# zc402/video-classification

Measured on AMD Instinct MI355X. Metric: clips/sec SlowFast-R50 8x8, 32x224^2 bf16 training step, higher is better.
Workload: dtype bf16

## Files before the change

### video-classification_amd/csrc/bn_tail.hip

```cpp
#include "sfk_common.h"

namespace {

template <typename D> __device__ __forceinline__ float wload(const void* w, int64_t i) {
  return (float)static_cast<const D*>(w)[i];
}

constexpr int TF_CO = 8;
constexpr int TF_MAXC = 512;

__global__ __launch_bounds__(256) void bn_tail_fold_g_kernel(const float* __restrict__ parts, int nparts, int c, float* __restrict__ g) {
  const int ci = blockIdx.x * 4 + (threadIdx.x >> 6), lane = threadIdx.x & 63;
  if (ci >= c) return;
  double s = 0.0;
  for (int p = lane; p < nparts; p += 64) s += (double)parts[((int64_t)p * c + ci) * 2];
#pragma unroll
  for (int sft = 1; sft < 64; sft <<= 1) s += __shfl_xor(s, sft);
  if (lane == 0) g[ci] = (float)s;
}

template <typename D>
__global__ __launch_bounds__(256) void bn_tail_fwd_kernel(const float* __restrict__ gram, const float* __restrict__ gvec,
                                                          double n, int c, const void* w,
                                                          int cout, const float* gamma, const float* beta, float eps,
                                                          float momentum, float* running_mean, float* running_var,
                                                          int64_t* nbt, float* mean, float* invstd, float* scale,
                                                          float* shift, float* __restrict__ t, D* __restrict__ wd) {
  __shared__ float wl[TF_CO][TF_MAXC];
  __shared__ float gl[TF_MAXC];
  __shared__ double red[4 * TF_CO][2];
  __shared__ float acoef[TF_CO];
  const int co0 = blockIdx.x * TF_CO, tid = threadIdx.x;
  if (blockIdx.x == 0 && tid == 0 && nbt) nbt[0] += 1;
  const double inv_n = 1.0 / n;
  for (int i = tid; i < TF_CO * c; i += 256) {
    const int o = i / c, j = i % c;
    wl[o][j] = co0 + o < cout ? wload<D>(w, (int64_t)(co0 + o) * c + j) : 0.f;
  }
  for (int j = tid; j < c; j += 256) gl[j] = (float)((double)gvec[j] * inv_n);
  __syncthreads();
  constexpr int NR = TF_MAXC / 256;
  float acc[TF_CO][NR], accc[TF_CO][NR];
  double gbar[NR];
#pragma unroll
  for (int r = 0; r < NR; ++r) {
    const int ci = tid + 256 * r;
    gbar[r] = ci < c ? (double)gvec[ci] * inv_n : 0.0;
  }
#pragma unroll
  for (int o = 0; o < TF_CO; ++o)
#pragma unroll
    for (int r = 0; r < NR; ++r) { acc[o][r] = 0.f; accc[o][r] = 0.f; }
#pragma unroll 8
  for (int j = 0; j < c; ++j) {
    float gj[NR], gc[NR];
    const double mj = (double)gl[j];
#pragma unroll
    for (int r = 0; r < NR; ++r) {
      const int ci = tid + 256 * r;
      gj[r] = ci < c ? gram[(int64_t)j * c + ci] : 0.f;
      gc[r] = (float)((double)gj[r] * inv_n - mj * gbar[r]);
    }
#pragma unroll
    for (int o = 0; o < TF_CO; ++o) {
      const float wv = wl[o][j];
#pragma unroll
      for (int r = 0; r < NR; ++r) {
        acc[o][r] += wv * gj[r];
        accc[o][r] += wv * gc[r];
      }
    }
  }
  double p1[TF_CO], p2[TF_CO];
#pragma unroll
  for (int o = 0; o < TF_CO; ++o) {
    p1[o] = 0.0;
    p2[o] = 0.0;
#pragma unroll
    for (int r = 0; r < NR; ++r) {
      const int ci = tid + 256 * r;
      if (ci < c) {
        if (co0 + o < cout) t[(int64_t)(co0 + o) * c + ci] = acc[o][r];
        p1[o] += (double)wl[o][ci] * (double)gvec[ci];
        p2[o] += (double)accc[o][r] * (double)wl[o][ci];
      }
    }
#pragma unroll
    for (int sft = 1; sft < 64; sft <<= 1) {
      p1[o] += __shfl_xor(p1[o], sft);
      p2[o] += __shfl_xor(p2[o], sft);
    }
  }
  if ((tid & 63) == 0) {
#pragma unroll
    for (int o = 0; o < TF_CO; ++o) {
      red[(tid >> 6) * TF_CO + o][0] = p1[o];
      red[(tid >> 6) * TF_CO + o][1] = p2[o];
    }
  }
  __syncthreads();
  if (tid < TF_CO && co0 + tid < cout) {
    const int ch = co0 + tid;
    const double s1 = red[tid][0] + red[TF_CO + tid][0] + red[2 * TF_CO + tid][0] + red[3 * TF_CO + tid][0];
    const double s2 = red[tid][1] + red[TF_CO + tid][1] + red[2 * TF_CO + tid][1] + red[3 * TF_CO + tid][1];
    const double mu = s1 / n;
    double var = s2;
    if (var < 0.0) var = 0.0;
    const float is = (float)(1.0 / sqrt(var + (double)eps));
    const float sc = gamma[ch] * is;
    mean[ch] = (float)mu;
    invstd[ch] = is;
    scale[ch] = sc;
    shift[ch] = beta[ch] - (float)mu * sc;
    acoef[tid] = sc;
    if (running_mean) {
      const double unb = n > 1.0 ? var * n / (n - 1.0) : var;
      running_mean[ch] = (1.f - momentum) * running_mean[ch] + momentum * (float)mu;
      running_var[ch] = (1.f - momentum) * running_var[ch] + momentum * (float)unb;
    }
  }
  if (!wd) return;
  __syncthreads();
  for (int ci = tid; ci < c; ci += 256)
#pragma unroll
    for (int o = 0; o < TF_CO; ++o)
      if (co0 + o < cout) wd[(int64_t)ci * cout + co0 + o] = (D)(acoef[o] * wl[o][ci]);
}

template <typename D>
__global__ __launch_bounds__(256) void bn_tail_coef_kernel(const float* __restrict__ rx, const float* __restrict__ parts,
                                                           int nparts, double n, int c,
                                                           const void* w, int cout, const float* gamma,
                                                           const float* mean, const float* invstd, float* dgamma,
                                                           float* dbeta, float* coef) {
  const int co = blockIdx.x * 4 + (threadIdx.x >> 6), lane = threadIdx.x & 63;
  if (co >= cout) return;
  double sdy = 0.0;
#pragma unroll 4
  for (int ci = lane; ci < c; ci += 64) sdy += (double)wload<D>(w, (int64_t)co * c + ci) * (double)rx[(int64_t)co * c + ci];
  double s = 0.0;
#pragma unroll 8
  for (int p = lane; p < nparts; p += 64) s += (double)parts[((int64_t)p * cout + co) * 2];
#pragma unroll
  for (int sft = 1; sft < 64; sft <<= 1) {
    sdy += __shfl_xor(sdy, sft);
    s += __shfl_xor(s, sft);
  }
  if (lane != 0) return;
  const double is = (double)invstd[co], mu = (double)mean[co];
  const double sxh = is * (sdy - mu * s);
  dgamma[co] += (float)sxh;
  dbeta[co] += (float)s;
  const double A = (double)gamma[co] * is, c1 = s / n, c2 = sxh / n;
  coef[co * 4 + 0] = (float)A;
  coef[co * 4 + 1] = (float)(-A * c2 * is);
  coef[co * 4 + 2] = (float)(A * (c2 * is * mu - c1));
  coef[co * 4 + 3] = 0.f;
}

template <typename D>
__device__ __forceinline__ void bn_tail_apply_part(int bx, int by, const float* __restrict__ rx, const float* __restrict__ gvec,
                                                   const float* __restrict__ t, int c, int cout,
                                                   const float* __restrict__ coef, float* dw) {
  const int co0 = by * 32, ci0 = bx * 32;
  const int tx = threadIdx.x & 31, ty = threadIdx.x >> 5;
#pragma unroll
  for (int i = 0; i < 4; ++i) {
    const int co = co0 + ty + 8 * i, ci = ci0 + tx;
    if (co < cout && ci < c) {
      const float A = coef[co * 4], B = coef[co * 4 + 1], Cc = coef[co * 4 + 2];
      const int64_t idx = (int64_t)co * c + ci;
      dw[idx] += A * rx[idx] + B * t[idx] + Cc * gvec[ci];
    }
  }
}

template <typename D>
__device__ __forceinline__ void bn_tail_m_part(int bx, int by, const void* w, int c, int cout, const float* __restrict__ coef, D* m) {
  __shared__ float wi[16][17], wj[16][17], bco[16];
  const int tx = threadIdx.x & 15, ty = threadIdx.x >> 4;
  const int i = by * 16 + ty, j = bx * 16 + tx;
  float acc = 0.f;
  for (int co0 = 0; co0 < cout; co0 += 16) {
    const int co = co0 + ty;
    const int ci = by * 16 + tx, cj = bx * 16 + tx;
    wi[ty][tx] = (co < cout && ci < c) ? wload<D>(w, (int64_t)co * c + ci) : 0.f;
    wj[ty][tx] = (co < cout && cj < c) ? wload<D>(w, (int64_t)co * c + cj) : 0.f;
    if (threadIdx.x < 16) bco[threadIdx.x] = co0 + threadIdx.x < cout ? coef[(co0 + threadIdx.x) * 4 + 1] : 0.f;
    __syncthreads();
#pragma unroll
    for (int q = 0; q < 16; ++q) acc += bco[q] * wi[q][ty] * wj[q][tx];
    __syncthreads();
  }
  if (i < c && j < c) m[(int64_t)i * c + j] = (D)acc;
}

template <typename D>
__device__ __forceinline__ void bn_tail_bias_part(int bx, const void* w, int c, int cout, const float* __restrict__ coef,
                                                  float* bias) {
  __shared__ double red[16][17];
  const int col = threadIdx.x & 15, part = threadIdx.x >> 4;
  const int ci = bx * 16 + col;
  double s = 0.0;
  if (ci < c) {
#pragma unroll 4
    for (int co = part; co < cout; co += 16) s += (double)coef[co * 4 + 2] * (double)wload<D>(w, (int64_t)co * c + ci);
  }
  red[part][col] = s;
  __syncthreads();
  if (part == 0 && ci < c) {
    double a = 0.0;
#pragma unroll
    for (int p = 0; p < 16; ++p) a += red[p][col];
    bias[ci] = (float)a;
  }
}

template <typename D>
__global__ __launch_bounds__(256) void bn_tail_post_kernel(const float* rx, const float* gvec, const float* t, int c,
                                                           const void* w, int cout, const float* coef, float* dw, D* m,
                                                           float* bias, int ax, int nap, int mx, int nm) {
  int b = blockIdx.x;
  if (b < nap) { bn_tail_apply_part<D>(b % ax, b / ax, rx, gvec, t, c, cout, coef, dw); return; }
  b -= nap;
  if (b < nm) { bn_tail_m_part<D>(b % mx, b / mx, w, c, cout, coef, m); return; }
  bn_tail_bias_part<D>(b - nm, w, c, cout, coef, bias);
}

inline bool tail_args_ok(int c, int cout, int dtype) {
  return c > 0 && cout > 0 && (dtype == SFK_F32 || dtype == SFK_BF16);
}

}

extern "C" int sfk_bn_tail_fwd(const float* gram, const float* a_sums, int32_t a_nparts, int64_t count, float* g, int32_t c,
                               const void* w, int32_t w_dtype, int32_t cout,
                               const float* gamma, const float* beta, float eps, float momentum, float* running_mean,
                               float* running_var, int64_t* nbt, float* mean, float* invstd, float* scale, float* shift,
                               float* t, void* wd, sfk_stream_t stream) {
  if (!gram || !a_sums || a_nparts <= 0 || count <= 0 || !g || !w || !gamma || !beta || !mean || !invstd || !scale || !shift || !t)
    return SFK_ERR_INVALID;
  if (!tail_args_ok(c, cout, w_dtype) || (!running_mean) != (!running_var)) return SFK_ERR_INVALID;
  if (c > TF_MAXC) return SFK_ERR_UNSUPPORTED;
  hipStream_t s = static_cast<hipStream_t>(stream);
  hipLaunchKernelGGL(bn_tail_fold_g_kernel, dim3((c + 3) / 4), dim3(256), 0, s, a_sums, a_nparts, c, g);
  const dim3 grid((cout + TF_CO - 1) / TF_CO), blk(256);
  if (w_dtype == SFK_BF16)
    hipLaunchKernelGGL(bn_tail_fwd_kernel<bf16_t>, grid, blk, 0, s, gram, g, (double)count, c, w, cout, gamma, beta, eps, momentum,
                       running_mean, running_var, nbt, mean, invstd, scale, shift, t, static_cast<bf16_t*>(wd));
  else
    hipLaunchKernelGGL(bn_tail_fwd_kernel<float>, grid, blk, 0, s, gram, g, (double)count, c, w, cout, gamma, beta, eps, momentum,
                       running_mean, running_var, nbt, mean, invstd, scale, shift, t, static_cast<float*>(wd));
  SFK_CHECK_LAUNCH();
  return SFK_OK;
}

template <typename D>
static int tail_bwd_launch(const float* rx, const float* parts, int nparts, const float* g, int64_t count, const float* t, int c, const void* w, int cout,
                           const float* gamma, const float* mean, const float* invstd, float* dgamma, float* dbeta,
                           float* dw, void* m, float* bias, float* coef, hipStream_t s) {
  hipLaunchKernelGGL(bn_tail_coef_kernel<D>, dim3((cout + 3) / 4), dim3(256), 0, s, rx, parts, nparts, (double)count, c, w, cout, gamma, mean,
                     invstd, dgamma, dbeta, coef);
  const int ax = (c + 31) / 32, ay = (cout + 31) / 32, mx = (c + 15) / 16, nb = (c + 15) / 16;
  hipLaunchKernelGGL(bn_tail_post_kernel<D>, dim3(ax * ay + mx * mx + nb), dim3(256), 0, s, rx, g, t, c, w, cout, coef, dw,
                     static_cast<D*>(m), bias, ax, ax * ay, mx, mx * mx);
  SFK_CHECK_LAUNCH();
  return SFK_OK;
}

extern "C" int sfk_bn_tail_bwd(const float* rx, const float* parts, int32_t nparts, const float* g, int64_t count, const float* t,
                               int32_t c, const void* w, int32_t w_dtype, int32_t cout, const float* gamma, const float* mean, const float* invstd,
                               float* dgamma, float* dbeta, float* dw, void* m, float* bias, float* coef,
                               sfk_stream_t stream) {
  if (!rx || !parts || nparts <= 0 || !g || count <= 0 || !t || !w || !gamma || !mean || !invstd || !dgamma || !dbeta || !dw || !m || !bias || !coef)
    return SFK_ERR_INVALID;
  if (!tail_args_ok(c, cout, w_dtype)) return SFK_ERR_INVALID;
  hipStream_t s = static_cast<hipStream_t>(stream);
  return w_dtype == SFK_BF16
             ? tail_bwd_launch<bf16_t>(rx, parts, nparts, g, count, t, c, w, cout, gamma, mean, invstd, dgamma, dbeta, dw, m, bias, coef, s)
             : tail_bwd_launch<float>(rx, parts, nparts, g, count, t, c, w, cout, gamma, mean, invstd, dgamma, dbeta, dw, m, bias, coef, s);
}
```

Before: 1167.

## Use fp32 MFMA for BN-tail gram products and coalesce partial-sum folds

Rewrites the BN-tail forward W·Gram product and the backward W^T·diag(B)·W product to use 16x16x4 fp32 MFMA instructions, with register double-buffered gram loads and templated column tiling chosen by channel count. The partial-sum fold kernels now reduce 8 channels per block with 32 loads in flight per thread, replacing one-wave-per-channel strided reads. The post-kernel block order is also changed so the heavier M blocks are scheduled first. The cost targeted is scalar FMA throughput and poorly coalesced reads in these small BN-tail kernels. In exchange the code is more complex, and accumulating in fp32 MFMA may change rounding order.

```diff
diff --git a/video-classification_amd/csrc/bn_tail.hip b/video-classification_amd/csrc/bn_tail.hip
--- a/video-classification_amd/csrc/bn_tail.hip
+++ b/video-classification_amd/csrc/bn_tail.hip
@@ -6,125 +6,181 @@
   return (float)static_cast<const D*>(w)[i];
 }
 
-constexpr int TF_CO = 8;
+constexpr int TF_CO = 16;
 constexpr int TF_MAXC = 512;
+constexpr int FOLD_CH = 8;
+constexpr int FOLD_RG = 32;
+
+__device__ __forceinline__ f32x4 mma4(float a, float b, const f32x4& acc) {
+  return __builtin_amdgcn_mfma_f32_16x16x4f32(a, b, acc, 0, 0, 0);
+}
+
+constexpr int FOLD_U = 32;
+struct FoldRegs { float v[FOLD_U]; };
+__device__ __forceinline__ void fold_issue(const float* __restrict__ parts, int nparts, int nch, int ch, int p0, FoldRegs& f) {
+#pragma unroll
+  for (int u = 0; u < FOLD_U; ++u) {
+    const int p = p0 + u * FOLD_RG;
+    f.v[u] = (ch < nch && p < nparts) ? parts[((int64_t)p * nch + ch) * 2] : 0.f;
+  }
+}
+__device__ __forceinline__ double fold_sum(const FoldRegs& f) {
+  double s = 0.0;
+#pragma unroll
+  for (int u = 0; u < FOLD_U; ++u) s += (double)f.v[u];
+  return s;
+}
+__device__ __forceinline__ double fold_rows(const float* __restrict__ parts, int nparts, int nch, int ch0, const FoldRegs& first) {
+  __shared__ double fred[4][FOLD_CH];
+  const int tid = threadIdx.x, chl = tid & (FOLD_CH - 1), rg = tid / FOLD_CH, ch = ch0 + chl;
+  double s = fold_sum(first);
+  for (int p0 = rg + FOLD_U * FOLD_RG; p0 < nparts; p0 += FOLD_U * FOLD_RG) {
+    FoldRegs f;
+    fold_issue(parts, nparts, nch, ch, p0, f);
+    s += fold_sum(f);
+  }
+#pragma unroll
+  for (int sft = FOLD_CH; sft < 64; sft <<= 1) s += __shfl_xor(s, sft);
+  if ((tid & 63) < FOLD_CH) fred[tid >> 6][chl] = s;
+  __syncthreads();
+  return tid < FOLD_CH ? (fred[0][tid] + fred[1][tid]) + (fred[2][tid] + fred[3][tid]) : 0.0;
+}
 
 __global__ __launch_bounds__(256) void bn_tail_fold_g_kernel(const float* __restrict__ parts, int nparts, int c, float* __restrict__ g) {
-  const int ci = blockIdx.x * 4 + (threadIdx.x >> 6), lane = threadIdx.x & 63;
-  if (ci >= c) return;
-  double s = 0.0;
-  for (int p = lane; p < nparts; p += 64) s += (double)parts[((int64_t)p * c + ci) * 2];
-#pragma unroll
-  for (int sft = 1; sft < 64; sft <<= 1) s += __shfl_xor(s, sft);
-  if (lane == 0) g[ci] = (float)s;
-}
-
-template <typename D>
+  const int ch0 = blockIdx.x * FOLD_CH;
+  FoldRegs f;
+  fold_issue(parts, nparts, c, ch0 + (threadIdx.x & (FOLD_CH - 1)), threadIdx.x / FOLD_CH, f);
+  const double s = fold_rows(parts, nparts, c, ch0, f);
+  const int ci = ch0 + threadIdx.x;
+  if (threadIdx.x < FOLD_CH && ci < c) g[ci] = (float)s;
+}
+
+template <typename D, int NT>
 __global__ __launch_bounds__(256) void bn_tail_fwd_kernel(const float* __restrict__ gram, const float* __restrict__ gvec,
                                                           double n, int c, const void* w,
                                                           int cout, const float* gamma, const float* beta, float eps,
                                                           float momentum, float* running_mean, float* running_var,
                                                           int64_t* nbt, float* mean, float* invstd, float* scale,
                                                           float* shift, float* __restrict__ t, D* __restrict__ wd) {
-  __shared__ float wl[TF_CO][TF_MAXC];
-  __shared__ float gl[TF_MAXC];
-  __shared__ double red[4 * TF_CO][2];
+  constexpr int CP = 64 * NT, LD = CP + 4;
+  constexpr int KU = NT <= 2 ? 16 : 32 / NT;
+  constexpr int KP = NT == 1 ? 2 : 1;
+  __shared__ float wl[TF_CO][LD];
+  __shared__ double gd[CP];
+  __shared__ double red[4][TF_CO];
+  __shared__ double mus[TF_CO];
   __shared__ float acoef[TF_CO];
-  const int co0 = blockIdx.x * TF_CO, tid = threadIdx.x;
+  const int tid = threadIdx.x, wave = tid >> 6, l = tid & 63, lr = l & 15, lq = l >> 4;
+  const int co0 = blockIdx.x * TF_CO;
   if (blockIdx.x == 0 && tid == 0 && nbt) nbt[0] += 1;
   const double inv_n = 1.0 / n;
-  for (int i = tid; i < TF_CO * c; i += 256) {
-    const int o = i / c, j = i % c;
-    wl[o][j] = co0 + o < cout ? wload<D>(w, (int64_t)(co0 + o) * c + j) : 0.f;
-  }
-  for (int j = tid; j < c; j += 256) gl[j] = (float)((double)gvec[j] * inv_n);
-  __syncthreads();
-  constexpr int NR = TF_MAXC / 256;
-  float acc[TF_CO][NR], accc[TF_CO][NR];
-  double gbar[NR];
-#pragma unroll
-  for (int r = 0; r < NR; ++r) {
-    const int ci = tid + 256 * r;
-    gbar[r] = ci < c ? (double)gvec[ci] * inv_n : 0.0;
-  }
-#pragma unroll
-  for (int o = 0; o < TF_CO; ++o)
-#pragma unroll
-    for (int r = 0; r < NR; ++r) { acc[o][r] = 0.f; accc[o][r] = 0.f; }
-#pragma unroll 8
-  for (int j = 0; j < c; ++j) {
-    float gj[NR], gc[NR];
-    const double mj = (double)gl[j];
-#pragma unroll
-    for (int r = 0; r < NR; ++r) {
-      const int ci = tid + 256 * r;
-      gj[r] = ci < c ? gram[(int64_t)j * c + ci] : 0.f;
-      gc[r] = (float)((double)gj[r] * inv_n - mj * gbar[r]);
-    }
-#pragma unroll
-    for (int o = 0; o < TF_CO; ++o) {
-      const float wv = wl[o][j];
-#pragma unroll
-      for (int r = 0; r < NR; ++r) {
-        acc[o][r] += wv * gj[r];
-        accc[o][r] += wv * gc[r];
+  const int ksteps = (c + 3) >> 2;
+  int col[NT];
+  double gbc[NT];
+#pragma unroll
+  for (int q = 0; q < NT; ++q) {
+    col[q] = 16 * (wave + 4 * q) + lr;
+    gbc[q] = col[q] < c ? (double)gvec[col[q]] * inv_n : 0.0;
+  }
+  const bool fin = tid < TF_CO && co0 + tid < cout;
+  const float gam = fin ? gamma[co0 + tid] : 0.f, bet = fin ? beta[co0 + tid] : 0.f;
+  const float rm0 = (fin && running_mean) ? running_mean[co0 + tid] : 0.f, rv0 = (fin && running_mean) ? running_var[co0 + tid] : 0.f;
+  float gcur[KU][NT], gnxt[KU][NT];
+  auto load_g = [&](const int s0, float (&gr)[KU][NT]) __attribute__((always_inline)) {
+#pragma unroll
+    for (int u = 0; u < KU; ++u) {
+      const int k = 4 * (s0 + u) + lq;
+#pragma unroll
+      for (int q = 0; q < NT; ++q) gr[u][q] = (k < c && col[q] < c) ? gram[(int64_t)k * c + col[q]] : 0.f;
+    }
+  };
+  load_g(0, gcur);
+  for (int i = tid; i < TF_CO * CP; i += 256) {
+    const int o = i / CP, j = i % CP;
+    wl[o][j] = (co0 + o < cout && j < c) ? wload<D>(w, (int64_t)(co0 + o) * c + j) : 0.f;
+  }
+  for (int j = tid; j < CP; j += 256) gd[j] = j < c ? (double)gvec[j] * inv_n : 0.0;
+  __syncthreads();
+  f32x4 acc[KP][NT], accc[KP][NT];
+#pragma unroll
+  for (int p = 0; p < KP; ++p)
+#pragma unroll
+    for (int q = 0; q < NT; ++q)
+#pragma unroll
+      for (int i = 0; i < 4; ++i) { acc[p][q][i] = 0.f; accc[p][q][i] = 0.f; }
+  for (int s0 = 0; s0 < ksteps; s0 += KU) {
+    const bool more = s0 + KU < ksteps;
+    if (more) load_g(s0 + KU, gnxt);
+#pragma unroll
+    for (int u = 0; u < KU; ++u) {
+      const int k = 4 * (s0 + u) + lq;
+      const float a = wl[lr][k];
+      const double mk = gd[k];
+#pragma unroll
+      for (int q = 0; q < NT; ++q) {
+        const float gj = gcur[u][q];
+        const float gc = (float)((double)gj * inv_n - mk * gbc[q]);
+        acc[u % KP][q] = mma4(a, gj, acc[u % KP][q]);
+        accc[u % KP][q] = mma4(a, gc, accc[u % KP][q]);
       }
     }
-  }
-  double p1[TF_CO], p2[TF_CO];
-#pragma unroll
-  for (int o = 0; o < TF_CO; ++o) {
-    p1[o] = 0.0;
-    p2[o] = 0.0;
-#pragma unroll
-    for (int r = 0; r < NR; ++r) {
-      const int ci = tid + 256 * r;
-      if (ci < c) {
-        if (co0 + o < cout) t[(int64_t)(co0 + o) * c + ci] = acc[o][r];
-        p1[o] += (double)wl[o][ci] * (double)gvec[ci];
-        p2[o] += (double)accc[o][r] * (double)wl[o][ci];
-      }
-    }
-#pragma unroll
-    for (int sft = 1; sft < 64; sft <<= 1) {
-      p1[o] += __shfl_xor(p1[o], sft);
-      p2[o] += __shfl_xor(p2[o], sft);
-    }
-  }
-  if ((tid & 63) == 0) {
-#pragma unroll
-    for (int o = 0; o < TF_CO; ++o) {
-      red[(tid >> 6) * TF_CO + o][0] = p1[o];
-      red[(tid >> 6) * TF_CO + o][1] = p2[o];
-    }
-  }
-  __syncthreads();
-  if (tid < TF_CO && co0 + tid < cout) {
+    if (more) {
+#pragma unroll
+      for (int u = 0; u < KU; ++u)
+#pragma unroll
+        for (int q = 0; q < NT; ++q) gcur[u][q] = gnxt[u][q];
+    }
+  }
+  double p2[4] = {0.0, 0.0, 0.0, 0.0};
+#pragma unroll
+  for (int q = 0; q < NT; ++q)
+#pragma unroll
+    for (int i = 0; i < 4; ++i) {
+      const int row = 4 * lq + i;
+      float tv = acc[0][q][i], tc = accc[0][q][i];
+      if constexpr (KP == 2) { tv += acc[1][q][i]; tc += accc[1][q][i]; }
+      if (co0 + row < cout && col[q] < c) t[(int64_t)(co0 + row) * c + col[q]] = tv;
+      p2[i] += (double)tc * (double)wl[row][col[q]];
+    }
+#pragma unroll
+  for (int i = 0; i < 4; ++i) {
+#pragma unroll
+    for (int sft = 1; sft < 16; sft <<= 1) p2[i] += __shfl_xor(p2[i], sft);
+    if (lr == 0) red[wave][4 * lq + i] = p2[i];
+  }
+  {
+    const int row = tid >> 4;
+    double s = 0.0;
+    for (int ci = lr; ci < c; ci += 16) s += (double)wl[row][ci] * gd[ci];
+#pragma unroll
+    for (int sft = 1; sft < 16; sft <<= 1) s += __shfl_xor(s, sft);
+    if (lr == 0) mus[row] = s;
+  }
+  __syncthreads();
+  if (fin) {
     const int ch = co0 + tid;
-    const double s1 = red[tid][0] + red[TF_CO + tid][0] + red[2 * TF_CO + tid][0] + red[3 * TF_CO + tid][0];
-    const double s2 = red[tid][1] + red[TF_CO + tid][1] + red[2 * TF_CO + tid][1] + red[3 * TF_CO + tid][1];
-    const double mu = s1 / n;
-    double var = s2;
+    const double mu = mus[tid];
+    double var = red[0][tid] + red[1][tid] + red[2][tid] + red[3][tid];
     if (var < 0.0) var = 0.0;
     const float is = (float)(1.0 / sqrt(var + (double)eps));
-    const float sc = gamma[ch] * is;
+    const float sc = gam * is;
     mean[ch] = (float)mu;
     invstd[ch] = is;
     scale[ch] = sc;
-    shift[ch] = beta[ch] - (float)mu * sc;
+    shift[ch] = bet - (float)mu * sc;
     acoef[tid] = sc;
     if (running_mean) {
       const double unb = n > 1.0 ? var * n / (n - 1.0) : var;
-      running_mean[ch] = (1.f - momentum) * running_mean[ch] + momentum * (float)mu;
-      running_var[ch] = (1.f - momentum) * running_var[ch] + momentum * (float)unb;
+      running_mean[ch] = (1.f - momentum) * rm0 + momentum * (float)mu;
+      running_var[ch] = (1.f - momentum) * rv0 + momentum * (float)unb;
     }
   }
   if (!wd) return;
   __syncthreads();
-  for (int ci = tid; ci < c; ci += 256)
-#pragma unroll
-    for (int o = 0; o < TF_CO; ++o)
-      if (co0 + o < cout) wd[(int64_t)ci * cout + co0 + o] = (D)(acoef[o] * wl[o][ci]);
+  for (int i = tid; i < c * TF_CO; i += 256) {
+    const int ci = i / TF_CO, o = i % TF_CO;
+    if (co0 + o < cout) wd[(int64_t)ci * cout + co0 + o] = (D)(acoef[o] * wl[o][ci]);
+  }
 }
 
 template <typename D>
@@ -133,25 +189,33 @@
                                                            const void* w, int cout, const float* gamma,
                                                            const float* mean, const float* invstd, float* dgamma,
                                                            float* dbeta, float* coef) {
-  const int co = blockIdx.x * 4 + (threadIdx.x >> 6), lane = threadIdx.x & 63;
-  if (co >= cout) return;
-  double sdy = 0.0;
+  __shared__ double sd[FOLD_CH];
+  const int co0 = blockIdx.x * FOLD_CH, tid = threadIdx.x;
+  FoldRegs f;
+  fold_issue(parts, nparts, cout, co0 + (tid & (FOLD_CH - 1)), tid / FOLD_CH, f);
+  const bool fin = tid < FOLD_CH && co0 + tid < cout;
+  const float isf = fin ? invstd[co0 + tid] : 0.f, muf = fin ? mean[co0 + tid] : 0.f, gam = fin ? gamma[co0 + tid] : 0.f;
+  const float dg0 = fin ? dgamma[co0 + tid] : 0.f, db0 = fin ? dbeta[co0 + tid] : 0.f;
+  {
+    const int co = co0 + (tid >> 5), j = tid & 31;
+    double a = 0.0;
+    if (co < cout) {
 #pragma unroll 4
-  for (int ci = lane; ci < c; ci += 64) sdy += (double)wload<D>(w, (int64_t)co * c + ci) * (double)rx[(int64_t)co * c + ci];
-  double s = 0.0;
-#pragma unroll 8
-  for (int p = lane; p < nparts; p += 64) s += (double)parts[((int64_t)p * cout + co) * 2];
-#pragma unroll
-  for (int sft = 1; sft < 64; sft <<= 1) {
-    sdy += __shfl_xor(sdy, sft);
-    s += __shfl_xor(s, sft);
-  }
-  if (lane != 0) return;
-  const double is = (double)invstd[co], mu = (double)mean[co];
+      for (int ci = j; ci < c; ci += 32) a += (double)wload<D>(w, (int64_t)co * c + ci) * (double)rx[(int64_t)co * c + ci];
+    }
+#pragma unroll
+    for (int sft = 1; sft < 32; sft <<= 1) a += __shfl_xor(a, sft);
+    if (j == 0) sd[tid >> 5] = a;
+  }
+  const double s = fold_rows(parts, nparts, cout, co0, f);
+  if (!fin) return;
+  const int co = co0 + tid;
+  const double sdy = sd[tid];
+  const double is = (double)isf, mu = (double)muf;
   const double sxh = is * (sdy - mu * s);
-  dgamma[co] += (float)sxh;
-  dbeta[co] += (float)s;
-  const double A = (double)gamma[co] * is, c1 = s / n, c2 = sxh / n;
+  dgamma[co] = dg0 + (float)sxh;
+  dbeta[co] = db0 + (float)s;
+  const double A = (double)gam * is, c1 = s / n, c2 = sxh / n;
   coef[co * 4 + 0] = (float)A;
   coef[co * 4 + 1] = (float)(-A * c2 * is);
   coef[co * 4 + 2] = (float)(A * (c2 * is * mu - c1));
@@ -177,22 +241,46 @@
 
 template <typename D>
 __device__ __forceinline__ void bn_tail_m_part(int bx, int by, const void* w, int c, int cout, const float* __restrict__ coef, D* m) {
-  __shared__ float wi[16][17], wj[16][17], bco[16];
-  const int tx = threadIdx.x & 15, ty = threadIdx.x >> 4;
-  const int i = by * 16 + ty, j = bx * 16 + tx;
-  float acc = 0.f;
-  for (int co0 = 0; co0 < cout; co0 += 16) {
-    const int co = co0 + ty;
-    const int ci = by * 16 + tx, cj = bx * 16 + tx;
-    wi[ty][tx] = (co < cout && ci < c) ? wload<D>(w, (int64_t)co * c + ci) : 0.f;
-    wj[ty][tx] = (co < cout && cj < c) ? wload<D>(w, (int64_t)co * c + cj) : 0.f;
-    if (threadIdx.x < 16) bco[threadIdx.x] = co0 + threadIdx.x < cout ? coef[(co0 + threadIdx.x) * 4 + 1] : 0.f;
-    __syncthreads();
-#pragma unroll
-    for (int q = 0; q < 16; ++q) acc += bco[q] * wi[q][ty] * wj[q][tx];
-    __syncthreads();
-  }
-  if (i < c && j < c) m[(int64_t)i * c + j] = (D)acc;
+  constexpr int KU = 16;
+  __shared__ float part[3][64][4];
+  const int tid = threadIdx.x, wave = tid >> 6, l = tid & 63, lr = l & 15, lq = l >> 4;
+  const int i = by * 16 + lr, j = bx * 16 + lr;
+  const int ksteps = (cout + 3) >> 2, per = (ksteps + 3) >> 2;
+  const int s_end = min(ksteps, (wave + 1) * per);
+  f32x4 acc[4];
+#pragma unroll
+  for (int p = 0; p < 4; ++p)
+#pragma unroll
+    for (int e = 0; e < 4; ++e) acc[p][e] = 0.f;
+  for (int s0 = wave * per; s0 < s_end; s0 += KU) {
+    float av[KU], bv[KU];
+#pragma unroll
+    for (int u = 0; u < KU; ++u) {
+      const int co = 4 * (s0 + u) + lq;
+      const bool ok = s0 + u < s_end && co < cout;
+      const float b = ok ? coef[co * 4 + 1] : 0.f;
+      const float wi = (ok && i < c) ? wload<D>(w, (int64_t)co * c + i) : 0.f;
+      av[u] = b * wi;
+      bv[u] = (ok && j < c) ? wload<D>(w, (int64_t)co * c + j) : 0.f;
+    }
+#pragma unroll
+    for (int u = 0; u < KU; ++u) acc[u & 3] = mma4(av[u], bv[u], acc[u & 3]);
+  }
+  f32x4 sum;
+#pragma unroll
+  for (int e = 0; e < 4; ++e) sum[e] = (acc[0][e] + acc[1][e]) + (acc[2][e] + acc[3][e]);
+  if (wave > 0) {
+#pragma unroll
+    for (int e = 0; e < 4; ++e) part[wave - 1][l][e] = sum[e];
+  }
+  __syncthreads();
+  if (wave > 0) return;
+#pragma unroll
+  for (int e = 0; e < 4; ++e) {
+    const float v = ((sum[e] + part[0][l][e]) + part[1][l][e]) + part[2][l][e];
+    const int row = by * 16 + 4 * lq + e;
+    if (row < c && j < c) m[(int64_t)row * c + j] = (D)v;
+  }
 }
 
 template <typename D>
@@ -203,7 +291,7 @@
   const int ci = bx * 16 + col;
   double s = 0.0;
   if (ci < c) {
-#pragma unroll 4
+#pragma unroll 8
     for (int co = part; co < cout; co += 16) s += (double)coef[co * 4 + 2] * (double)wload<D>(w, (int64_t)co * c + ci);
   }
   red[part][col] = s;
@@ -221,10 +309,10 @@
                                                            const void* w, int cout, const float* coef, float* dw, D* m,
                                                            float* bias, int ax, int nap, int mx, int nm) {
   int b = blockIdx.x;
+  if (b < nm) { bn_tail_m_part<D>(b % mx, b / mx, w, c, cout, coef, m); return; }
+  b -= nm;
   if (b < nap) { bn_tail_apply_part<D>(b % ax, b / ax, rx, gvec, t, c, cout, coef, dw); return; }
-  b -= nap;
-  if (b < nm) { bn_tail_m_part<D>(b % mx, b / mx, w, c, cout, coef, m); return; }
-  bn_tail_bias_part<D>(b - nm, w, c, cout, coef, bias);
+  bn_tail_bias_part<D>(b - nap, w, c, cout, coef, bias);
 }
 
 inline bool tail_args_ok(int c, int cout, int dtype) {
@@ -232,6 +320,17 @@
 }
 
 }
+
+template <typename D, int NT>
+static void tail_fwd_launch(const float* gram, const float* g, int64_t count, int c, const void* w, int cout, const float* gamma,
+                            const float* beta, float eps, float momentum, float* running_mean, float* running_var, int64_t* nbt,
+                            float* mean, float* invstd, float* scale, float* shift, float* t, void* wd, hipStream_t s) {
+  hipLaunchKernelGGL((bn_tail_fwd_kernel<D, NT>), dim3((cout + TF_CO - 1) / TF_CO), dim3(256), 0, s, gram, g, (double)count, c, w,
+                     cout, gamma, beta, eps, momentum, running_mean, running_var, nbt, mean, invstd, scale, shift, t,
+                     static_cast<D*>(wd));
+}
+#define SFK_TAIL_FWD_ARGS \
+  gram, g, count, c, w, cout, gamma, beta, eps, momentum, running_mean, running_var, nbt, mean, invstd, scale, shift, t, wd, s
 
 extern "C" int sfk_bn_tail_fwd(const float* gram, const float* a_sums, int32_t a_nparts, int64_t count, float* g, int32_t c,
                                const void* w, int32_t w_dtype, int32_t cout,
@@ -243,14 +342,13 @@
   if (!tail_args_ok(c, cout, w_dtype) || (!running_mean) != (!running_var)) return SFK_ERR_INVALID;
   if (c > TF_MAXC) return SFK_ERR_UNSUPPORTED;
   hipStream_t s = static_cast<hipStream_t>(stream);
-  hipLaunchKernelGGL(bn_tail_fold_g_kernel, dim3((c + 3) / 4), dim3(256), 0, s, a_sums, a_nparts, c, g);
-  const dim3 grid((cout + TF_CO - 1) / TF_CO), blk(256);
-  if (w_dtype == SFK_BF16)
-    hipLaunchKernelGGL(bn_tail_fwd_kernel<bf16_t>, grid, blk, 0, s, gram, g, (double)count, c, w, cout, gamma, beta, eps, momentum,
-                       running_mean, running_var, nbt, mean, invstd, scale, shift, t, static_cast<bf16_t*>(wd));
-  else
-    hipLaunchKernelGGL(bn_tail_fwd_kernel<float>, grid, blk, 0, s, gram, g, (double)count, c, w, cout, gamma, beta, eps, momentum,
-                       running_mean, running_var, nbt, mean, invstd, scale, shift, t, static_cast<float*>(wd));
+  hipLaunchKernelGGL(bn_tail_fold_g_kernel, dim3((c + FOLD_CH - 1) / FOLD_CH), dim3(256), 0, s, a_sums, a_nparts, c, g);
+  const bool bf = w_dtype == SFK_BF16;
+  const int nt = c <= 64 ? 1 : c <= 128 ? 2 : c <= 256 ? 4 : 8;
+  if (nt == 1) bf ? tail_fwd_launch<bf16_t, 1>(SFK_TAIL_FWD_ARGS) : tail_fwd_launch<float, 1>(SFK_TAIL_FWD_ARGS);
+  else if (nt == 2) bf ? tail_fwd_launch<bf16_t, 2>(SFK_TAIL_FWD_ARGS) : tail_fwd_launch<float, 2>(SFK_TAIL_FWD_ARGS);
+  else if (nt == 4) bf ? tail_fwd_launch<bf16_t, 4>(SFK_TAIL_FWD_ARGS) : tail_fwd_launch<float, 4>(SFK_TAIL_FWD_ARGS);
+  else bf ? tail_fwd_launch<bf16_t, 8>(SFK_TAIL_FWD_ARGS) : tail_fwd_launch<float, 8>(SFK_TAIL_FWD_ARGS);
   SFK_CHECK_LAUNCH();
   return SFK_OK;
 }
@@ -259,7 +357,7 @@
 static int tail_bwd_launch(const float* rx, const float* parts, int nparts, const float* g, int64_t count, const float* t, int c, const void* w, int cout,
                            const float* gamma, const float* mean, const float* invstd, float* dgamma, float* dbeta,
                            float* dw, void* m, float* bias, float* coef, hipStream_t s) {
-  hipLaunchKernelGGL(bn_tail_coef_kernel<D>, dim3((cout + 3) / 4), dim3(256), 0, s, rx, parts, nparts, (double)count, c, w, cout, gamma, mean,
+  hipLaunchKernelGGL(bn_tail_coef_kernel<D>, dim3((cout + FOLD_CH - 1) / FOLD_CH), dim3(256), 0, s, rx, parts, nparts, (double)count, c, w, cout, gamma, mean,
                      invstd, dgamma, dbeta, coef);
   const int ax = (c + 31) / 32, ay = (cout + 31) / 32, mx = (c + 15) / 16, nb = (c + 15) / 16;
   hipLaunchKernelGGL(bn_tail_post_kernel<D>, dim3(ax * ay + mx * mx + nb), dim3(256), 0, s, rx, g, t, c, w, cout, coef, dw,
```

New measurement: 1167. No clear change (-0.0%).

## Add LDS-resident gram path for small-channel BN tail and widen reductions

Applied to the files above, without the earlier changes.

For channel counts up to 128, a new forward kernel stages the whole gram matrix and a slab of weights in dynamic LDS and assigns each thread a column with two output channels. This replaces the generic per-8-channel kernel on that path. The partial-sum folds in the g and coef kernels now use 1024-thread blocks that reduce 16 channels across 64 row lanes, giving coalesced reads. The M-matrix part loads 256-channel slabs with register prefetch instead of 16-row tiles. These changes aim to cut global re-reads and sync overhead in the small BN tail kernels, at the cost of larger LDS use (possibly above 64KB via attribute) and more code paths.

```diff
diff --git a/video-classification_amd/csrc/bn_tail.hip b/video-classification_amd/csrc/bn_tail.hip
--- a/video-classification_amd/csrc/bn_tail.hip
+++ b/video-classification_amd/csrc/bn_tail.hip
@@ -8,15 +8,141 @@
 
 constexpr int TF_CO = 8;
 constexpr int TF_MAXC = 512;
-
-__global__ __launch_bounds__(256) void bn_tail_fold_g_kernel(const float* __restrict__ parts, int nparts, int c, float* __restrict__ g) {
-  const int ci = blockIdx.x * 4 + (threadIdx.x >> 6), lane = threadIdx.x & 63;
-  if (ci >= c) return;
+constexpr int TF_LDSC = 128;
+constexpr int TF_CPT = 2;
+
+constexpr int FR_CH = 16;
+constexpr int FR_ROWS = 64;
+
+__device__ __forceinline__ double fold_rows(const float* __restrict__ parts, int nparts, int nch, int ch0, double* red) {
+  const int tid = threadIdx.x, cl = tid & (FR_CH - 1), rl = tid / FR_CH, ch = ch0 + cl;
   double s = 0.0;
-  for (int p = lane; p < nparts; p += 64) s += (double)parts[((int64_t)p * c + ci) * 2];
-#pragma unroll
-  for (int sft = 1; sft < 64; sft <<= 1) s += __shfl_xor(s, sft);
-  if (lane == 0) g[ci] = (float)s;
+  if (ch < nch) {
+#pragma unroll 16
+    for (int p = rl; p < nparts; p += FR_ROWS) s += (double)parts[((int64_t)p * nch + ch) * 2];
+  }
+  s += __shfl_xor(s, 16);
+  s += __shfl_xor(s, 32);
+  if ((tid & 63) < FR_CH) red[(tid >> 6) * FR_CH + cl] = s;
+  __syncthreads();
+  double a = 0.0;
+  if (tid < FR_CH) {
+#pragma unroll
+    for (int wv = 0; wv < FR_ROWS / 4; ++wv) a += red[wv * FR_CH + tid];
+  }
+  return a;
+}
+
+__global__ __launch_bounds__(1024) void bn_tail_fold_g_kernel(const float* __restrict__ parts, int nparts, int c, float* __restrict__ g) {
+  __shared__ double red[FR_CH * FR_ROWS / 4];
+  const double s = fold_rows(parts, nparts, c, blockIdx.x * FR_CH, red);
+  const int ci = blockIdx.x * FR_CH + threadIdx.x;
+  if (threadIdx.x < FR_CH && ci < c) g[ci] = (float)s;
+}
+
+__device__ __forceinline__ float bn_tail_stats(int ch, double s1, double s2, double n, const float* gamma, const float* beta,
+                                               float eps, float momentum, float* running_mean, float* running_var, float* mean,
+                                               float* invstd, float* scale, float* shift) {
+  const double mu = s1 / n;
+  double var = s2;
+  if (var < 0.0) var = 0.0;
+  const float is = (float)(1.0 / sqrt(var + (double)eps));
+  const float sc = gamma[ch] * is;
+  mean[ch] = (float)mu;
+  invstd[ch] = is;
+  scale[ch] = sc;
+  shift[ch] = beta[ch] - (float)mu * sc;
+  if (running_mean) {
+    const double unb = n > 1.0 ? var * n / (n - 1.0) : var;
+    running_mean[ch] = (1.f - momentum) * running_mean[ch] + momentum * (float)mu;
+    running_var[ch] = (1.f - momentum) * running_var[ch] + momentum * (float)unb;
+  }
+  return sc;
+}
+
+template <typename D>
+__global__ __launch_bounds__(256) void bn_tail_fwd_lds_kernel(const float* __restrict__ gram, const float* __restrict__ gvec,
+                                                              double n, int c, int cw, const void* w,
+                                                              int cout, const float* gamma, const float* beta, float eps,
+                                                              float momentum, float* running_mean, float* running_var,
+                                                              int64_t* nbt, float* mean, float* invstd, float* scale,
+                                                              float* shift, float* __restrict__ t, D* __restrict__ wd) {
+  extern __shared__ __attribute__((aligned(16))) char smem[];
+  const int cob = 256 / cw * TF_CPT;
+  float* gs = reinterpret_cast<float*>(smem);
+  float* wl = gs + ((c * c + 3) & ~3);
+  float* gl = wl + cob * c;
+  float* acoef = gl + c;
+  double* red = reinterpret_cast<double*>(acoef + cob + ((c + cob * c) & 1));
+  const int tid = threadIdx.x, grp = tid / cw, ci = tid % cw;
+  const int co0 = blockIdx.x * cob, og = grp * TF_CPT;
+  if (blockIdx.x == 0 && tid == 0 && nbt) nbt[0] += 1;
+  const double inv_n = 1.0 / n;
+  const int gn = c * c;
+  if ((gn & 3) == 0 && (reinterpret_cast<uintptr_t>(gram) & 15) == 0) {
+    const float4* g4 = reinterpret_cast<const float4*>(gram);
+    for (int i = tid; i < gn / 4; i += 256) reinterpret_cast<float4*>(gs)[i] = g4[i];
+  } else {
+    for (int i = tid; i < gn; i += 256) gs[i] = gram[i];
+  }
+  for (int i = tid; i < cob * c; i += 256) {
+    const int o = i / c;
+    wl[i] = co0 + o < cout ? wload<D>(w, (int64_t)co0 * c + i) : 0.f;
+  }
+  for (int j = tid; j < c; j += 256) gl[j] = (float)((double)gvec[j] * inv_n);
+  const bool live = ci < c;
+  const double gsum = live ? (double)gvec[ci] : 0.0, gbar = gsum * inv_n;
+  __syncthreads();
+  float acc[TF_CPT], accc[TF_CPT];
+#pragma unroll
+  for (int k = 0; k < TF_CPT; ++k) { acc[k] = 0.f; accc[k] = 0.f; }
+  const float* wrow = wl + og * c;
+#pragma unroll 8
+  for (int j = 0; j < c; ++j) {
+    const float gj = live ? gs[j * c + ci] : 0.f;
+    const float gc = (float)((double)gj * inv_n - (double)gl[j] * gbar);
+#pragma unroll
+    for (int k = 0; k < TF_CPT; ++k) {
+      const float wv = wrow[k * c + j];
+      acc[k] += wv * gj;
+      accc[k] += wv * gc;
+    }
+  }
+  const int sub = cw < 64 ? cw : 64, nsub = cw / sub;
+#pragma unroll
+  for (int k = 0; k < TF_CPT; ++k) {
+    double p1 = 0.0, p2 = 0.0;
+    if (live) {
+      const float wv = wrow[k * c + ci];
+      if (co0 + og + k < cout) t[(int64_t)(co0 + og + k) * c + ci] = acc[k];
+      p1 = (double)wv * gsum;
+      p2 = (double)accc[k] * (double)wv;
+    }
+    for (int sft = 1; sft < sub; sft <<= 1) {
+      p1 += __shfl_xor(p1, sft);
+      p2 += __shfl_xor(p2, sft);
+    }
+    if ((ci & (sub - 1)) == 0) {
+      red[((og + k) * 2 + ci / sub) * 2] = p1;
+      red[((og + k) * 2 + ci / sub) * 2 + 1] = p2;
+    }
+  }
+  __syncthreads();
+  if (tid < cob) {
+    float sc = 0.f;
+    if (co0 + tid < cout) {
+      double s1 = red[tid * 4], s2 = red[tid * 4 + 1];
+      if (nsub == 2) { s1 += red[tid * 4 + 2]; s2 += red[tid * 4 + 3]; }
+      sc = bn_tail_stats(co0 + tid, s1, s2, n, gamma, beta, eps, momentum, running_mean, running_var, mean, invstd, scale, shift);
+    }
+    acoef[tid] = sc;
+  }
+  if (!wd) return;
+  __syncthreads();
+  for (int i = tid; i < cob * c; i += 256) {
+    const int o = i % cob, cc = i / cob;
+    if (co0 + o < cout) wd[(int64_t)cc * cout + co0 + o] = (D)(acoef[o] * wl[o * c + cc]);
+  }
 }
 
 template <typename D>
@@ -100,24 +226,9 @@
   }
   __syncthreads();
   if (tid < TF_CO && co0 + tid < cout) {
-    const int ch = co0 + tid;
     const double s1 = red[tid][0] + red[TF_CO + tid][0] + red[2 * TF_CO + tid][0] + red[3 * TF_CO + tid][0];
     const double s2 = red[tid][1] + red[TF_CO + tid][1] + red[2 * TF_CO + tid][1] + red[3 * TF_CO + tid][1];
-    const double mu = s1 / n;
-    double var = s2;
-    if (var < 0.0) var = 0.0;
-    const float is = (float)(1.0 / sqrt(var + (double)eps));
-    const float sc = gamma[ch] * is;
-    mean[ch] = (float)mu;
-    invstd[ch] = is;
-    scale[ch] = sc;
-    shift[ch] = beta[ch] - (float)mu * sc;
-    acoef[tid] = sc;
-    if (running_mean) {
-      const double unb = n > 1.0 ? var * n / (n - 1.0) : var;
-      running_mean[ch] = (1.f - momentum) * running_mean[ch] + momentum * (float)mu;
-      running_var[ch] = (1.f - momentum) * running_var[ch] + momentum * (float)unb;
-    }
+    acoef[tid] = bn_tail_stats(co0 + tid, s1, s2, n, gamma, beta, eps, momentum, running_mean, running_var, mean, invstd, scale, shift);
   }
   if (!wd) return;
   __syncthreads();
@@ -128,25 +239,29 @@
 }
 
 template <typename D>
-__global__ __launch_bounds__(256) void bn_tail_coef_kernel(const float* __restrict__ rx, const float* __restrict__ parts,
-                                                           int nparts, double n, int c,
-                                                           const void* w, int cout, const float* gamma,
-                                                           const float* mean, const float* invstd, float* dgamma,
-                                                           float* dbeta, float* coef) {
-  const int co = blockIdx.x * 4 + (threadIdx.x >> 6), lane = threadIdx.x & 63;
-  if (co >= cout) return;
-  double sdy = 0.0;
+__global__ __launch_bounds__(1024) void bn_tail_coef_kernel(const float* __restrict__ rx, const float* __restrict__ parts,
+                                                            int nparts, double n, int c,
+                                                            const void* w, int cout, const float* gamma,
+                                                            const float* mean, const float* invstd, float* dgamma,
+                                                            float* dbeta, float* coef) {
+  __shared__ double red[FR_CH * FR_ROWS / 4];
+  __shared__ double dot[FR_CH];
+  const int co0 = blockIdx.x * FR_CH, lane = threadIdx.x & 63;
+  {
+    const int co = co0 + (threadIdx.x >> 6);
+    double sdy = 0.0;
+    if (co < cout) {
 #pragma unroll 4
-  for (int ci = lane; ci < c; ci += 64) sdy += (double)wload<D>(w, (int64_t)co * c + ci) * (double)rx[(int64_t)co * c + ci];
-  double s = 0.0;
-#pragma unroll 8
-  for (int p = lane; p < nparts; p += 64) s += (double)parts[((int64_t)p * cout + co) * 2];
-#pragma unroll
-  for (int sft = 1; sft < 64; sft <<= 1) {
-    sdy += __shfl_xor(sdy, sft);
-    s += __shfl_xor(s, sft);
-  }
-  if (lane != 0) return;
+      for (int ci = lane; ci < c; ci += 64) sdy += (double)wload<D>(w, (int64_t)co * c + ci) * (double)rx[(int64_t)co * c + ci];
+    }
+#pragma unroll
+    for (int sft = 1; sft < 64; sft <<= 1) sdy += __shfl_xor(sdy, sft);
+    if (lane == 0) dot[threadIdx.x >> 6] = sdy;
+  }
+  const double s = fold_rows(parts, nparts, cout, co0, red);
+  const int co = co0 + threadIdx.x;
+  if (threadIdx.x >= FR_CH || co >= cout) return;
+  const double sdy = dot[threadIdx.x];
   const double is = (double)invstd[co], mu = (double)mean[co];
   const double sxh = is * (sdy - mu * s);
   dgamma[co] += (float)sxh;
@@ -175,21 +290,39 @@
   }
 }
 
+constexpr int TM_SLAB = 256;
+
 template <typename D>
 __device__ __forceinline__ void bn_tail_m_part(int bx, int by, const void* w, int c, int cout, const float* __restrict__ coef, D* m) {
-  __shared__ float wi[16][17], wj[16][17], bco[16];
+  __shared__ float wi[TM_SLAB][16], wj[TM_SLAB][16], bco[TM_SLAB];
+  constexpr int NL = TM_SLAB / 16;
   const int tx = threadIdx.x & 15, ty = threadIdx.x >> 4;
   const int i = by * 16 + ty, j = bx * 16 + tx;
+  const int ci = by * 16 + tx, cj = bx * 16 + tx;
+  float ri[NL], rj[NL], rb;
+  auto fetch = [&](int co0) {
+#pragma unroll
+    for (int l = 0; l < NL; ++l) {
+      const int co = co0 + ty + 16 * l;
+      ri[l] = (co < cout && ci < c) ? wload<D>(w, (int64_t)co * c + ci) : 0.f;
+      rj[l] = (co < cout && cj < c) ? wload<D>(w, (int64_t)co * c + cj) : 0.f;
+    }
+    rb = co0 + (int)threadIdx.x < cout ? coef[(co0 + threadIdx.x) * 4 + 1] : 0.f;
+  };
+  fetch(0);
   float acc = 0.f;
-  for (int co0 = 0; co0 < cout; co0 += 16) {
-    const int co = co0 + ty;
-    const int ci = by * 16 + tx, cj = bx * 16 + tx;
-    wi[ty][tx] = (co < cout && ci < c) ? wload<D>(w, (int64_t)co * c + ci) : 0.f;
-    wj[ty][tx] = (co < cout && cj < c) ? wload<D>(w, (int64_t)co * c + cj) : 0.f;
-    if (threadIdx.x < 16) bco[threadIdx.x] = co0 + threadIdx.x < cout ? coef[(co0 + threadIdx.x) * 4 + 1] : 0.f;
+  for (int co0 = 0; co0 < cout; co0 += TM_SLAB) {
+#pragma unroll
+    for (int l = 0; l < NL; ++l) {
+      wi[ty + 16 * l][tx] = ri[l];
+      wj[ty + 16 * l][tx] = rj[l];
+    }
+    bco[threadIdx.x] = rb;
     __syncthreads();
-#pragma unroll
-    for (int q = 0; q < 16; ++q) acc += bco[q] * wi[q][ty] * wj[q][tx];
+    if (co0 + TM_SLAB < cout) fetch(co0 + TM_SLAB);
+    const int nq = min(TM_SLAB, (cout - co0 + 15) & ~15);
+#pragma unroll 16
+    for (int q = 0; q < nq; ++q) acc += bco[q] * wi[q][ty] * wj[q][tx];
     __syncthreads();
   }
   if (i < c && j < c) m[(int64_t)i * c + j] = (D)acc;
@@ -203,7 +336,7 @@
   const int ci = bx * 16 + col;
   double s = 0.0;
   if (ci < c) {
-#pragma unroll 4
+#pragma unroll 8
     for (int co = part; co < cout; co += 16) s += (double)coef[co * 4 + 2] * (double)wload<D>(w, (int64_t)co * c + ci);
   }
   red[part][col] = s;
@@ -231,6 +364,33 @@
   return c > 0 && cout > 0 && (dtype == SFK_F32 || dtype == SFK_BF16);
 }
 
+}
+
+template <typename D>
+static int tail_fwd_launch(const float* gram, const float* g, int64_t count, int c, const void* w, int cout, const float* gamma,
+                           const float* beta, float eps, float momentum, float* running_mean, float* running_var, int64_t* nbt,
+                           float* mean, float* invstd, float* scale, float* shift, float* t, void* wd, hipStream_t s) {
+  if (c > TF_LDSC) {
+    hipLaunchKernelGGL(bn_tail_fwd_kernel<D>, dim3((cout + TF_CO - 1) / TF_CO), dim3(256), 0, s, gram, g, (double)count, c, w, cout,
+                       gamma, beta, eps, momentum, running_mean, running_var, nbt, mean, invstd, scale, shift, t, static_cast<D*>(wd));
+    return SFK_OK;
+  }
+  int cw = 8;
+  while (cw < c) cw <<= 1;
+  const int cob = 256 / cw * TF_CPT;
+  const size_t floats = (size_t)((c * c + 3) & ~3) + (size_t)cob * c + c + cob + 1;
+  const size_t lds = floats * 4 + (size_t)cob * 4 * sizeof(double);
+  static bool raised = false;
+  if (lds > 65536 && !raised) {
+    if (hipFuncSetAttribute(reinterpret_cast<const void*>(&bn_tail_fwd_lds_kernel<D>), hipFuncAttributeMaxDynamicSharedMemorySize,
+                            (int)(((size_t)TF_LDSC * TF_LDSC + 8 * TF_LDSC) * 4)) != hipSuccess)
+      return SFK_ERR_LAUNCH;
+    raised = true;
+  }
+  hipLaunchKernelGGL(bn_tail_fwd_lds_kernel<D>, dim3((cout + cob - 1) / cob), dim3(256), lds, s, gram, g, (double)count, c, cw, w,
+                     cout, gamma, beta, eps, momentum, running_mean, running_var, nbt, mean, invstd, scale, shift, t,
+                     static_cast<D*>(wd));
+  return SFK_OK;
 }
 
 extern "C" int sfk_bn_tail_fwd(const float* gram, const float* a_sums, int32_t a_nparts, int64_t count, float* g, int32_t c,
@@ -243,14 +403,13 @@
   if (!tail_args_ok(c, cout, w_dtype) || (!running_mean) != (!running_var)) return SFK_ERR_INVALID;
   if (c > TF_MAXC) return SFK_ERR_UNSUPPORTED;
   hipStream_t s = static_cast<hipStream_t>(stream);
-  hipLaunchKernelGGL(bn_tail_fold_g_kernel, dim3((c + 3) / 4), dim3(256), 0, s, a_sums, a_nparts, c, g);
-  const dim3 grid((cout + TF_CO - 1) / TF_CO), blk(256);
-  if (w_dtype == SFK_BF16)
-    hipLaunchKernelGGL(bn_tail_fwd_kernel<bf16_t>, grid, blk, 0, s, gram, g, (double)count, c, w, cout, gamma, beta, eps, momentum,
-                       running_mean, running_var, nbt, mean, invstd, scale, shift, t, static_cast<bf16_t*>(wd));
-  else
-    hipLaunchKernelGGL(bn_tail_fwd_kernel<float>, grid, blk, 0, s, gram, g, (double)count, c, w, cout, gamma, beta, eps, momentum,
-                       running_mean, running_var, nbt, mean, invstd, scale, shift, t, static_cast<float*>(wd));
+  hipLaunchKernelGGL(bn_tail_fold_g_kernel, dim3((c + FR_CH - 1) / FR_CH), dim3(1024), 0, s, a_sums, a_nparts, c, g);
+  const int rc = w_dtype == SFK_BF16
+                     ? tail_fwd_launch<bf16_t>(gram, g, count, c, w, cout, gamma, beta, eps, momentum, running_mean, running_var, nbt, mean,
+                                               invstd, scale, shift, t, wd, s)
+                     : tail_fwd_launch<float>(gram, g, count, c, w, cout, gamma, beta, eps, momentum, running_mean, running_var, nbt, mean,
+                                              invstd, scale, shift, t, wd, s);
+  if (rc != SFK_OK) return rc;
   SFK_CHECK_LAUNCH();
   return SFK_OK;
 }
@@ -259,7 +418,7 @@
 static int tail_bwd_launch(const float* rx, const float* parts, int nparts, const float* g, int64_t count, const float* t, int c, const void* w, int cout,
                            const float* gamma, const float* mean, const float* invstd, float* dgamma, float* dbeta,
                            float* dw, void* m, float* bias, float* coef, hipStream_t s) {
-  hipLaunchKernelGGL(bn_tail_coef_kernel<D>, dim3((cout + 3) / 4), dim3(256), 0, s, rx, parts, nparts, (double)count, c, w, cout, gamma, mean,
+  hipLaunchKernelGGL(bn_tail_coef_kernel<D>, dim3((cout + FR_CH - 1) / FR_CH), dim3(1024), 0, s, rx, parts, nparts, (double)count, c, w, cout, gamma, mean,
                      invstd, dgamma, dbeta, coef);
   const int ax = (c + 31) / 32, ay = (cout + 31) / 32, mx = (c + 15) / 16, nb = (c + 15) / 16;
   hipLaunchKernelGGL(bn_tail_post_kernel<D>, dim3(ax * ay + mx * mx + nb), dim3(256), 0, s, rx, g, t, c, w, cout, coef, dw,
```

After: 1165 before, 1167 after, median of 6. Within noise of the previous version (+0.2%).
